# xiyichen/morphablediffusion

Hardware: AMD Instinct MI355X
Metric: multi-view denoising steps/sec (N=16 views, 256x256, CFG 2.0, DDIM-50 step) (higher is better)
Workload: dtype f16; 1 GPU; synthetic sample (FaceScape-FLAME-sized mesh, 5023 vertices before voxel de-duplication): N=16 target views, 256x256 (latent 32x32), perspective cameras, full-width UNet (916.9M params, random init), CFG 2.0, one denoise_apply per step; views_per_gpu=16, batch_view_num=16, parallelism=single GPU

## Files before the change

include/mvd.h:

```cpp
#ifndef MVD_H
#define MVD_H
#include <stddef.h>
#include <stdint.h>

#ifdef __cplusplus
extern "C" {
#endif

typedef struct mvd_ctx mvd_ctx;

typedef struct {
  int image_size;
  int in_channels;
  int out_channels;
  int model_channels;
  int num_res_blocks;
  int channel_mult[4];
  int num_heads;
  int context_dim;
  int volume_dims[4];
  int attention_levels;
} mvd_unet_config;

typedef struct {
// ... 132 lines not shown
int mvd_denoise_views_ms(mvd_ctx* ctx, int B, const int* slots, const float* x_noisy, const float* x_input, const float* clip,
                         const int64_t* timesteps, const float* t_embed, const float* v_embed, const int32_t* view_idx, int TN,
                         float cfg_scale, const float* noise, float s1m, float sqrt_at, float c_x, float c_d, float c_c, float c_n,
                         float* x0_hist, int first, float* eps_out, float* x_next, void* stream);

int mvd_op_cfg_ms(const float* eps_c, const float* eps_u, float scale, const float* x, const float* noise, float s1m, float sqrt_at,
                  float c_x, float c_d, float c_c, float c_n, float* x0_hist, int first, float* eps_out, float* x_next, size_t n,
                  void* stream);
int mvd_op_adamw_ex(float* p, const float* g, float* m, float* v, float* e, size_t n, float lr, float beta1, float beta2, float eps,
                    float wd, int step, float inv_scale, float max_grad_norm, float ema_decay, float* norm_out, void* stream);
int mvd_op_conv(mvd_ctx* ctx, const float* x_nchw, int B, int Cin, int H, int W, const float* w, const float* bias,
                int Cout, int ksize, int stride, int upsample, const float* resid_nchw, float* out_nchw, int force_splitk,
                void* stream);
int mvd_op_linear(mvd_ctx* ctx, const float* a, int M, int K, const float* w, const float* bias, int N, int geglu,
                  const float* resid, int a_half, int force_splitk, float* out, void* stream);
int mvd_op_group_norm(mvd_ctx* ctx, const float* x_nchw, int B, int C, int HW, int groups, const float* gamma,
                      const float* beta, float eps, int act, float* out_nchw, void* stream);
int mvd_op_layer_norm(mvd_ctx* ctx, const float* x, int rows, int C, const float* gamma, const float* beta, float* out,
                      void* stream);
int mvd_op_attention(mvd_ctx* ctx, const float* q, const float* k, const float* v, int B, int T, int heads, int d,
                     float* out, void* stream);
int mvd_op_depth_attn(mvd_ctx* ctx, const float* qk, const float* context, const float* fill_row, int n_cond, int HW, int D, int Cc,
                      int heads, int ldx, int split, int nfill, int check_only, float* out, float* hi_out, void* stream);
int mvd_op_conv3d(mvd_ctx* ctx, const float* x_ncdhw, int B, int Cin, int D, int H, int W, const float* w,
                  const float* bias, int Cout, int stride, int transposed, const float* resid, float* out, void* stream);
int mvd_op_attention_bwd(mvd_ctx* ctx, const float* q, const float* k, const float* v, const float* d_out, int B, int T, int heads,
                         int d, float* dq, float* dk, float* dv, void* stream);
int mvd_op_group_norm_bwd(mvd_ctx* ctx, const float* x, const float* dy, int B, int rows, int C, int groups, const float* gamma,
                          const float* beta, float eps, int act, float* dx, float* dgamma, float* dbeta, void* stream);
int mvd_op_layer_norm_bwd(mvd_ctx* ctx, const float* x, const float* dy, int rows, int C, const float* gamma, float* dx,
                          float* dgamma, float* dbeta, void* stream);
int mvd_op_conv_bwd(mvd_ctx* ctx, int kind, int ksize, int B, int Cin, int H, int W, int Cout, const float* x, int x_f16,
                    const float* w, const float* dy, int xp, int accum, int need_din, int poison, float* dx, float* dw, float* db,
                    void* stream);
int mvd_op_linear_bwd(mvd_ctx* ctx, int B, int rows, int K, int N, const float* x, int x_f16, const float* w, const float* bias,
                      const float* dy, int geglu, int dx_f16, int staged, int xp, int accum, int poison, float* dx, float* dw,
                      float* db, void* stream);
int mvd_op_conv3d_bwd(mvd_ctx* ctx, int kind, int B, int Cin, int D, int H, int W, int Cout, const float* x, int x_f16,
                      const float* w, const float* dy, int accum, int poison, float* dx, float* dw, float* db, void* stream);
int mvd_op_tgemm(mvd_ctx* ctx, int M, int N, int K, const float* a, int a_f16, int a_trans, long lda, const float* b, int b_f16,
                 int b_trans, long ldb, float* out, int ldc, int accum, int xp, int poison, void* stream);
int mvd_op_st_tail(mvd_ctx* ctx, int C, int rows, int T, const float* ao, const float* xin, const float* rowbias,
                   const float* w_ao, const float* b_ao, const float* ln_g, const float* ln_b, const float* w1, const float* b1,
                   const float* w2, const float* b2, const float* w_po, const float* b_po, const float* resid, float* out,
                   int flags, int iters, float* ms_out, void* stream);
int mvd_op_st_head(mvd_ctx* ctx, int rows, int xp, const float* n0, const float* w_pi, const float* b_pi, const float* ln_g,
// ... 17 lines not shown
```

morphablediffusion_amd/csrc/c_api.hip:

```cpp
#include <array>
#include <dlfcn.h>
#include <stdlib.h>
#include <string.h>

#include <algorithm>
#include <string>
#include <utility>
#include <vector>

#include "engine.h"
#include "rowchain.h"

static thread_local std::string g_err;
int mvd_fail(const char* msg) {
  g_err = msg ? msg : "unknown error";
  return -1;
}
const char* mvd_error_text() { return g_err.c_str(); }

namespace {

__global__ void split_rows_to_f32_kernel(const half_t* in, int rows, int C, float* out) {
  for (size_t i = (size_t)blockIdx.x * blockDim.x + threadIdx.x; i < (size_t)rows * C; i += (size_t)gridDim.x * blockDim.x) {
    const size_t r = i / C, c = i % C;
// ... 1312 lines not shown
  split = split ? 1 : 0;
  const int W4 = 4 * Cc, wz = split ? 3 : 1;
  const size_t npix = (size_t)n_cond * HW, rows = npix + nfill, crows = npix * D;
  half_t* cn = ws_alloc<half_t>(c, crows * ldx + 8);
  half_t* z = ws_alloc<half_t>(c, (rows + 1) * W4 * wz);
  half_t* fr = ws_alloc<half_t>(c, (size_t)W4 * 3);
  WS_CHECK(cn && z && fr);
  HIP_CHECK_RET(hipMemsetAsync(cn, 0xFF, (crows * ldx + 8) * sizeof(half_t), s));
  HIP_CHECK_RET(hipMemsetAsync(z, 0xFF, (rows + 1) * W4 * wz * sizeof(half_t), s));
  if (crows) hipLaunchKernelGGL(rows_f32_to_f16_ld_kernel, dim3(nblk(crows * Cc)), dim3(256), 0, s, context, crows, Cc, cn, ldx);
  if (nfill > 0) {
    if (split) RET_IF(launch_rows_f32_to_f16_split(fill_row, W4, 1, W4, fr, s));
    else RET_IF(launch_f32_to_f16(fill_row, fr, W4, s));
  }
  RET_IF(launch_depth_attn(qk, cn, z, n_cond, HW, D, Cc, heads, s, split, nfill, nfill > 0 ? fr : nullptr, ldx));
  const size_t n = (rows + 1) * W4;
  if (split) {
    hipLaunchKernelGGL(split_rows_to_f32_kernel, dim3(nblk(n)), dim3(256), 0, s, z, (int)(rows + 1), W4, out);
    if (hi_out) hipLaunchKernelGGL(rows_f16_ld_to_f32_kernel, dim3(nblk(n)), dim3(256), 0, s, z, rows + 1, W4, 3 * W4, hi_out);
  } else {
    hipLaunchKernelGGL(f16_to_f32_kernel, dim3(nblk(n)), dim3(256), 0, s, z, out, n);
  }
  HIP_CHECK_RET(hipGetLastError());
  return 0;
}

int mvd_op_attention_bwd(mvd_ctx* c, const float* q, const float* k, const float* v, const float* d_out, int B, int T, int heads, int d,
                         float* dq, float* dk, float* dv, void* stream) {
  if (c && hipSetDevice(c->device) != hipSuccess) return mvd_fail("hipSetDevice failed");
  if (!c) return mvd_fail("null context");
  hipStream_t s = S(stream);
  WsScope ws_scope(c);
  const int C = heads * d, rows = B * T;
  half_t* qkv = ws_alloc<half_t>(c, (size_t)rows * 3 * C);
  half_t* o = ws_alloc<half_t>(c, (size_t)rows * C);
  half_t* do16 = ws_alloc<half_t>(c, (size_t)rows * C);
  half_t* dqkv = ws_alloc<half_t>(c, (size_t)rows * 3 * C);
  float* lse = ws_alloc<float>(c, (size_t)B * heads * T);
  float* delta = ws_alloc<float>(c, (size_t)B * heads * T);
  float* tmp = ws_alloc<float>(c, (size_t)rows * 3 * C);
  WS_CHECK(qkv && o && do16 && dqkv && lse && delta && tmp);
  hipLaunchKernelGGL(pack_qkv_rows_kernel, dim3(nblk((size_t)rows * C)), dim3(256), 0, s, q, k, v, rows, C, qkv);
  RET_IF(launch_attention(qkv, 3 * C, qkv + 2 * C, 3 * C, o, C, B, T, heads, d, s));
  RET_IF(bwd_cast_rows(d_out, C, rows, C, C, do16, s));
  RET_IF(bwd_attention(qkv, 3 * C, o, do16, C, dqkv, 3 * C, lse, delta, B, T, heads, d, s));
  hipLaunchKernelGGL(f16_to_f32_kernel, dim3(nblk((size_t)rows * 3 * C)), dim3(256), 0, s, dqkv, tmp, (size_t)rows * 3 * C);
// ... 375 lines not shown
```

morphablediffusion_amd/csrc/common.h:

```cpp
#pragma once
#include <hip/hip_runtime.h>
#include <hip/hip_fp16.h>
#include <stdint.h>

#include "env.h"

#ifdef MVD_BF16
typedef __bf16 half_t;
#define MVD_MFMA_32x32x16 __builtin_amdgcn_mfma_f32_32x32x16_bf16
#define MVD_MFMA_16x16x32 __builtin_amdgcn_mfma_f32_16x16x32_bf16
#define MVD_DTYPE_NAME "bf16"
#else
typedef _Float16 half_t;
#define MVD_MFMA_32x32x16 __builtin_amdgcn_mfma_f32_32x32x16_f16
#define MVD_MFMA_16x16x32 __builtin_amdgcn_mfma_f32_16x16x32_f16
#define MVD_DTYPE_NAME "f16"
#endif
typedef half_t h8 __attribute__((ext_vector_type(8)));
typedef half_t h4 __attribute__((ext_vector_type(4)));
typedef half_t h2 __attribute__((ext_vector_type(2)));
typedef float f32x16 __attribute__((ext_vector_type(16)));
typedef float f32x4 __attribute__((ext_vector_type(4)));

#define MVD_MAX_TAPS 27
// ... 116 lines not shown
int launch_gn_group(const float* x, int ld, int B, int rows, int C, int G, const float* preadd, int pld, const float* gamma,
                    const float* beta, float eps, int act, half_t* out, int ldo, hipStream_t s, int split = 0,
                    int nslab = 1, size_t slab_stride = 0, const float* bias2 = nullptr, const float* resid = nullptr, int ldr = 0,
                    float* mat = nullptr, int ldm = 0);
int launch_layernorm(const float* x, int rows, int C, const float* gamma, const float* beta, float eps,
                     half_t* out, hipStream_t s, half_t* raw = nullptr, int ld_raw = 0);
bool layernorm_slabs_takes(int C);
int launch_layernorm_slabs(const float* slabs, int nslab, size_t slab_stride, int rows, int C, const float* bias, const float* rowbias,
                           int rb_ld, int T, const float* resid, int ldr, float* mat, const float* gamma, const float* beta, float eps,
                           half_t* out, hipStream_t s, half_t* raw = nullptr, int ld_raw = 0);
int launch_layernorm_f32(const float* x, long ldx, int rows, int C, const float* gamma, const float* beta, float eps,
                         float* out, hipStream_t s);
int launch_attention(const half_t* qk, int ldqk, const half_t* v, int ldv, half_t* out, int ldo, int B, int T, int heads,
                     int d, hipStream_t s, int Tstride = 0);
int launch_clip_patches(const float* img, int B, int H, int W, int S, int P, int Kp, half_t* out, hipStream_t s);
int launch_clip_tokens(const float* pe, const float* cls, const float* pos, int B, int T, int Tp, int C, float* x,
                       hipStream_t s);
int launch_scale_copy(const float* src, size_t n, float k, float* dst, hipStream_t s);
int launch_softmax_rows(const float* s, long rows, int cols, half_t* p, hipStream_t st);
int launch_softmax_rows_f32(const float* s, long rows, int cols, float* p, hipStream_t st);
int launch_depth_attn(const float* qk, const half_t* ctxn, half_t* z, int n_cond, int HW, int D, int Cc, int heads,
                      hipStream_t s, int split = 0, int nfill = 0, const half_t* fill_row = nullptr, int ldx = 0);
int depth_attn_check(int D, int Cc, int heads, int ldx, int nfill);
int launch_small_linear(const float* a, int lda, int rows, int K, const half_t* w, const float* bias, int N,
                        int act_in, float* out, int ldo, int accumulate, hipStream_t s);
int launch_timestep_embedding(const int64_t* t, int B, int dim, float* out, hipStream_t s);
int launch_nchw_to_nhwc(const float* in, int B, int C, int HW, float* out, int ldo, int cpad, hipStream_t s);
int launch_nhwc_to_nchw(const float* in, int ld, int B, int C, int HW, float* out, hipStream_t s);
int launch_pack_weight(const float* src, int N, int Cin, int taps, int transposed, int geglu, half_t* dst,
                       hipStream_t s, int cin_src = -1, int xp = 0);
int launch_rows_f32_to_f16_split(const float* in, int lda, long rows, int C, half_t* out, hipStream_t s);
int launch_permute_geglu_bias(const float* src, int N, float* dst, hipStream_t s);
int launch_f32_to_f16(const float* in, half_t* out, size_t n, hipStream_t s);
int launch_rows_f32_to_f16(const float* in, int lda, long rows, int C, half_t* out, hipStream_t s);
int launch_pack_upconv_weight(const float* src, int N, int Cin, half_t* dst, hipStream_t s);
int launch_fill_rows_f16(half_t* out, int ld, int rows, const half_t* vec, int n, hipStream_t s);
int launch_fold_qk(const float* wq, const float* wk, int heads, int hd, int Cc, int I, float scale, half_t* out,
                   hipStream_t s, float* out32 = nullptr);
int launch_fold_ov(const float* wo, const float* wv, int heads, int hd, int Cc, int I, half_t* out, hipStream_t s,
                   float* out32 = nullptr);
int launch_fold_mm(const float* a, int lda, const float* b, int ldb, int M, int N, int K, half_t* out16, int ldc, float* out32,
                   hipStream_t s);
int launch_relu_beta_tile(const float* beta, int Cc, int heads, half_t* out, hipStream_t s, int split = 0);
int launch_cfg_ddim(const float* eps_c, const float* eps_u, float scale, const float* x, const float* noise,
                    float sqrt_one_minus_at, float sqrt_at, float sqrt_aprev, float dir_coef, float sigma,
                    float* eps_out, float* x_prev, size_t n, hipStream_t s);
// ... 127 lines not shown
```

morphablediffusion_amd/csrc/engine_unet.hip:

```cpp
#include <string.h>

#include <algorithm>

#include "engine.h"

namespace {

void igemm_init(IGemm& g) {
  memset(&g, 0, sizeof(g));
  g.alpha = 1.0f;
  g.sz = g.sy = g.sx = 1;
  g.out_linear = 1;
  g.Z = g.Y = g.X = g.B = 1;
  g.IZ = g.IY = g.IX = 1;
  g.PZ = g.PY = g.PX = 1;
  for (int i = 0; i < MVD_MAX_TAPS; ++i) g.tap[i] = igemm_tap(0, 0, 0, i);
}

void igemm_fill(IGemm& g, const GemmArgs& ga) {
  g.a = ga.a;
  g.a_f32 = ga.a_f32;
  g.lda = ga.lda;
  g.Cin = ga.w->Cin;
  g.cin_alg = ga.w->xp ? ga.w->cin_l : ga.w->Cin;
// ... 752 lines not shown
  half_t* z = ws_alloc<half_t>(c, (size_t)rows * 4 * Cc * wz);
  float* o = ws_alloc<float>(c, (size_t)rows * I);
  float* o2 = ws_alloc<float>(c, (size_t)rows * I);
  WS_CHECK(p && pn && z && o && o2);
  const size_t slab_elems = (size_t)rows * I;
  auto offer_slabs = [&](GemmArgs& ga, int* sk, int ldo) {
    *sk = 1;
    if (!mvd_env().cond_defer || f.train || !gn_group_eligible(I, HW, I, 8, 0, ldo)) return;
    const size_t nsl = rows > 8192 ? 4 : 16;
    ga.slabs = ws_alloc<float>(c, nsl * slab_elems);
    ga.slabs_cap = ga.slabs ? nsl * slab_elems : 0;
    ga.sk_used = sk;
  };
  GemmArgs g;
  int skd = 1;
  g.a = in.p; g.a_f32 = 1; g.lda = in.ld; g.w = &d.proj_in; g.out = p; g.ldc = I;
  offer_slabs(g, &skd, xq ? 3 * I : I);
  RET_IF(run_linear(c, g, Bx, rows, f.s));
  if (skd > 1)
    RET_IF(run_group_norm(c, g.slabs, I, Bx, HW, d.gn_in, 8, 1e-5f, ACT_SILU, nullptr, pn, xq ? 3 * I : I, f.s, 0, xq, skd, slab_elems,
                          d.proj_in.bias));
  else
    RET_IF(run_group_norm(c, p, I, Bx, HW, d.gn_in, 8, 1e-5f, ACT_SILU, nullptr, pn, xq ? 3 * I : I, f.s, 0, xq));
  if (f.n_ctx > 0) {
    float* qk = ws_alloc<float>(c, (size_t)crow * 4 * Cc);
    half_t* cn = cond_idx >= 0 && f.cn_pre[cond_idx] ? nullptr : ws_alloc<half_t>(c, (size_t)crow * D * Cc);
    WS_CHECK(qk && (cn || (cond_idx >= 0 && f.cn_pre[cond_idx])));
    g = GemmArgs();
    g.a = pn; g.lda = xq ? 3 * I : I; g.w = &d.wqk; g.out = qk; g.ldc = 4 * Cc; g.use_bias = false;
    RET_IF(run_linear(c, g, f.n_ctx, crow, f.s));
    const half_t* cnp = cond_idx >= 0 ? f.cn_pre[cond_idx] : nullptr;
    if (cnp) {
      HIP_CHECK_RET(hipStreamWaitEvent(f.s, c->ev_cond[cond_idx], 0));
      cn = const_cast<half_t*>(cnp);
    } else if (ctx_fold_ok(f, d, HW, D, level)) {
      if (f.ctx_side) HIP_CHECK_RET(hipStreamWaitEvent(f.s, c->ev_ctx, 0));
      RET_IF(ctx_fold(f, d, HW, D, level, cn, f.s));
    } else {
      if (f.ctx_side) HIP_CHECK_RET(hipStreamWaitEvent(f.s, c->ev_ctx, 0));
      float* pc = ws_alloc<float>(c, (size_t)crow * D * Cc);
      WS_CHECK(pc);
      g = GemmArgs();
      g.a = f.src[level].p; g.a_f32 = f.src[level].f32; g.lda = Cc; g.w = &d.proj_ctx; g.out = pc; g.ldc = Cc; g.use_bias = false;
      RET_IF(run_linear(c, g, f.n_ctx, crow * D, f.s));
      RET_IF(run_group_norm(c, pc, Cc, f.n_ctx, D * HW, d.gn_ctx, 8, 1e-5f, ACT_RELU, nullptr, cn, Cc, f.s));
    }
    {
      ProbeScope ps(c, f.s, "depth_attn_kernel", 4.0 * crow * (double)D * 4 * Cc,
                    (double)crow * D * Cc * 2.0 + (double)crow * 4 * Cc * 6.0);
      RET_IF(launch_depth_attn(qk, cn, z, f.n_ctx, HW, D, Cc, 4, f.s, xo, rows - crow, d.relu_beta, cnp ? f.cn_ld[cond_idx] : Cc));
    }
  } else if (Bx > f.n_ctx) {
    RET_IF(launch_fill_rows_f16(z + (size_t)crow * 4 * Cc * wz, 4 * Cc * wz, rows - crow, d.relu_beta, 4 * Cc * wz, f.s));
  }
  g = GemmArgs();
  g.a = z; g.lda = 4 * Cc * wz; g.w = &d.wov; g.out = o; g.ldc = I; g.use_bias = false;
  offer_slabs(g, &skd, x1 ? 3 * I : I);
  RET_IF(run_linear(c, g, Bx, rows, f.s));
  if (skd > 1)
    RET_IF(run_group_norm(c, g.slabs, I, Bx, HW, d.gn_o1, 8, 1e-5f, ACT_RELU, nullptr, pn, x1 ? 3 * I : I, f.s, 0, x1, skd, slab_elems));
  else
    RET_IF(run_group_norm(c, o, I, Bx, HW, d.gn_o1, 8, 1e-5f, ACT_RELU, nullptr, pn, x1 ? 3 * I : I, f.s, 0, x1));
  g = GemmArgs();
  g.a = pn; g.lda = x1 ? 3 * I : I; g.w = &d.conv1; g.out = o2; g.ldc = I; g.use_bias = false;
  offer_slabs(g, &skd, x2 ? 3 * I : I);
  RET_IF(run_conv2d(c, g, Bx, H, W, 1, 0, f.s));
  if (skd > 1)
    RET_IF(run_group_norm(c, g.slabs, I, Bx, HW, d.gn_o2, 8, 1e-5f, ACT_RELU, nullptr, pn, x2 ? 3 * I : I, f.s, 0, x2, skd, slab_elems));
  else
    RET_IF(run_group_norm(c, o2, I, Bx, HW, d.gn_o2, 8, 1e-5f, ACT_RELU, nullptr, pn, x2 ? 3 * I : I, f.s, 0, x2));
  g = GemmArgs();
  g.a = pn; g.lda = x2 ? 3 * I : I; g.w = &d.conv2; g.out = out.p; g.ldc = out.ld; g.use_bias = false; g.resid = in.p; g.ldr = in.ld;
  RET_IF(run_conv2d(c, g, Bx, H, W, 1, 0, f.s));
  if (use_const) {
    ProbeScope ps(c, f.s, "cond_const_add", 0.0, (double)n_free * HW * d.dim * 8.0);
    RET_IF(launch_add_image_rows(in.p + (size_t)crow * in.ld, in.ld, c->cond_const[cond_idx].k, d.dim, n_free, HW,
                                 out.p + (size_t)crow * out.ld, out.ld, f.s));
  }
  return 0;
}

// ... 532 lines not shown
```

morphablediffusion_amd/csrc/env.h:

```cpp
#pragma once

#define MVD_ENV_TABLE(PROCESS, ENGINE, CALL, PROCESS_CALL) \
   \
  ENGINE(off, halo, "MVD_NO_HALO", true, "3x3 convs on the gather kernel instead of the LDS-halo / conv3x kernels") \
  PROCESS_CALL(off, conv3x, "MVD_NO_CONV3X", true, "no conv3x fragment streams: 3x3 ResBlock convs on the LDS-halo kernel") \
  PROCESS(off, up_conv3x, "MVD_NO_UP_CONV3X", true, "the 4x4 -> 8x8 upsample conv as the 9-tap GEMM on the fp32 source, not upsample + conv3x") \
  PROCESS(off, gemm_dma, "MVD_NO_GEMM_DMA", true, "GEMMs / 1x1 convs on the older register-staged igemm kernel, not the LDS-DMA kernel") \
  PROCESS(num, dense_min_m, "MVD_DENSE_MIN_M", 64, "fewest rows routed to the LDS-DMA kernel (2 views per rank: 7.08 ms at 512, 6.97 ms at 64)") \
  PROCESS(off, plain, "MVD_NO_PLAIN", true, "general row mapping for plain GEMMs instead of the PLAIN instantiations") \
  PROCESS(on, old_plan, "MVD_OLD_PLAN", false, "k-step cost model (gemm_dma_plan) instead of gemm_dma_plan_us for plain GEMMs") \
  PROCESS(on, igemm_f32_bn128, "MVD_IGEMM_F32_BN128", false, "fp32 sources on 128-column tiles where 160 is picked (32768 x 960 x 320: 48 vs 37 us)") \
  PROCESS(on, bm128, "MVD_BM128", false, "offer the planner the four-wave 128-row tiles: measured, lost (profiles/r06_b_bm_sweep.txt)") \
  PROCESS(on, bm128_off, "MVD_NO_BM128", false, "overrides MVD_BM128: the 128-row tiles stay off") \
  PROCESS(num, dense_bn, "MVD_DENSE_BN", 0, "sweep (tools/gemm_plan_sweep.py): column-tile width of the dense launches, 0 = planner's") \
  PROCESS(num, dense_sk, "MVD_DENSE_SK", 0, "sweep: split-K of the dense launches, 0 = planner's") \
  PROCESS(num, dense_bm, "MVD_DENSE_BM", 0, "sweep: 128 = four-wave row tiles with MVD_DENSE_BN, else 256") \
  PROCESS(num, halo_bn, "MVD_HALO_BN", 0, "sweep (tools/conv_bench3.py): column width of the LDS-halo kernel, 0 = planner's") \
  PROCESS(num, halo_sk, "MVD_HALO_SK", 0, "sweep: split over 64-channel chunks of the LDS-halo kernel, 0 = planner's") \
  PROCESS(off, parity_batch, "MVD_NO_PARITY_BATCH", true, "one launch per output-parity class of the transposed / upsample convs, not one for all") \
  PROCESS(num, par_walk_min, "MVD_PAR_WALK_MIN", 0, "tiles from which a workgroup walks the parity classes, 0 = never (profiles/r06_y_ab_pwalk.txt: nothing)") \
  PROCESS(off, xcd_cols, "MVD_NO_XCD_COLS", true, "row-tile-major XCD walk always, never the column-major one (common.h: xcd_prefers_cols)") \
  PROCESS(off, attn_xcd, "MVD_ATTN_NO_XCD", true, "attention with the pre-remap workgroup order") \
   \
  PROCESS(num, defer_max, "MVD_DEFER_MAX", 16, "largest split a consumer takes as slabs (4 = the round-3 limit)") \
  PROCESS(off, defer_reduce, "MVD_NO_DEFER_REDUCE", true, "ResBlock conv1 with its own reduce pass; also turns off ln_defer and cond_defer") \
  PROCESS(off, cond_defer, "MVD_NO_COND_DEFER", true, "the DepthTransformer's GEMMs in front of a GroupNorm with their reduce passes") \
  PROCESS(on, ln_defer, "MVD_LN_DEFER", false, "LayerNorm sums the split-K slabs of proj_in / to_out (profiles/r06_g_ab_ln_defer.txt: no time gained)") \
  PROCESS(off, carry, "MVD_NO_CARRY", true, "a block's last GEMM reduces its own slabs instead of leaving them to the next block's GroupNorm") \
   \
  PROCESS(on, gn_two_pass, "MVD_GN_TWO_PASS", false, "two-pass GroupNorm everywhere; also turns off defer_reduce, cond_defer and out_conv_f32") \
  PROCESS(on, skip_side, "MVD_SKIP_SIDE", false, "the ResBlock's 1x1 skip conv on a helper stream (profiles/r06_z_ab_skip_side.txt: nothing)") \
  PROCESS(off, rowchain, "MVD_NO_ROWCHAIN", true, "the transformer block behind the attention as layered GEMMs, not the row-chain kernel") \
  PROCESS(num, rowchain_min_rows, "MVD_ROWCHAIN_MIN_ROWS", 16384, "fewest rows that take the row-chain kernel") \
  PROCESS(off, rowhead, "MVD_NO_ROWHEAD", true, "proj_in, LayerNorm1 and q | k | v as separate launches, not the row-head kernel") \
  PROCESS(off, xp_fuse, "MVD_NO_XP_FUSE", true, "extended-precision proj_in / proj_out as separate GEMMs beside the row kernels") \
  PROCESS(off, ffp, "MVD_NO_FFP", true, "FF2 and proj_out as two GEMMs, not one over [gg | t2]") \
  PROCESS(on, ln_scalar, "MVD_LN_SCALAR", false, "element-per-thread LayerNorm (also keeps FF2 and proj_out apart)") \
  PROCESS(off, ctx_fold, "MVD_NO_CTX_FOLD", true, "GroupNorm(proj_context(volume)) materialised, not folded into two GEMM passes") \
  PROCESS(off, ctx_group, "MVD_NO_CTX_GROUP", true, "context fold block by block, not once per level") \
  PROCESS(off, cond_const, "MVD_NO_COND_CONST", true, "DepthTransformer over all samples, context-free ones included (profiles/r06_i_ab_cond_const.txt)") \
  PROCESS(off, conv_in_f32, "MVD_NO_CONV_IN_F32", true, "the input conv on the MFMA forms, not in exact fp32 on the vector ALU") \
  PROCESS(off, out_conv_f32, "MVD_NO_OUT_CONV_F32", true, "the output head on the MFMA forms, not GroupNorm + conv in exact fp32") \
  PROCESS(off, side_stream, "MVD_NO_SIDE_STREAM", true, "context volumes and folds on the caller's stream") \
  PROCESS(off, side_emb, "MVD_NO_SIDE_EMB", true, "the timestep-embedding GEMMs on the caller's stream") \
  PROCESS(on, one_way_fork, "MVD_ONE_WAY_FORK", false, "side-stream fork without the acknowledgement: the round-1 race on demand (DESIGN.md section 4, tools/det_fork.sh)") \
   \
  PROCESS(off, fused_enc, "MVD_NO_FUSED_ENC", true, "the 2-D target encoder layer by layer, not as one launch") \
  CALL(one, bn_loop, "MVD_BN_LOOP", false, "the looped BatchNorm + ReLU kernel; tests/test_gpu_train.py flips it for its bit-identity check") \
  CALL(one, sparse_valu, "MVD_SPARSE_VALU", false, "read when sparse-conv weights are built: one-site-per-workgroup kernels and the scatter-form data gradient") \
  CALL(num, xp, "MVD_XP", precision_level, "overrides the engine's extended-precision level when the policy is applied") \
  PROCESS(on, stage_scalar, "MVD_STAGE_SCALAR", false, "element-per-thread staging kernels of the backward pass (profiles/r04_m_*)") \
  PROCESS(on, gn_bwd_one_block, "MVD_GN_BWD_ONE_BLOCK", false, "mvd_op_group_norm_bwd: one workgroup per (sample, group), not the slabbed form") \
  PROCESS(one, repack_one_stream, "MVD_REPACK_STREAMS", false, "=1: the training re-pack on one stream, not four") \
   \
  PROCESS(on, plan_debug, "MVD_PLAN_DEBUG", false, "print every dense plan as a [plan] line") \
  PROCESS(on, layer_timing, "MVD_LAYER_TIMING", false, "per-GEMM event time (tools/layer_step.py); synchronises every launch") \
  PROCESS(on, debug_sum, "MVD_DEBUG_SUM", false, "bit checksums of the step's buffers: which differ between repeats?") \
  PROCESS(on, mesh_timing, "MVD_MESH_TIMING", false, "host phases of set_mesh / set_samples") \
  PROCESS(on, cond_bwd_timing, "MVD_COND_BWD_TIMING", false, "host-side enqueue time of each conditioner-backward phase")

#include <stdlib.h>

// ... 45 lines not shown
```

morphablediffusion_amd/engine.py:

```python
import collections
import ctypes as C
import os
from typing import Dict, Optional

import torch

from . import lib as L
from .spec import UNetConfig, VolumeConfig


def _stream():
    return torch.cuda.current_stream().cuda_stream


def _f32(t, device):
    return t.detach().to(device=device, dtype=torch.float32).contiguous()


IncompatibleKeys = collections.namedtuple("IncompatibleKeys", ["missing_keys", "unexpected_keys"])
MAX_SAMPLE_SLOTS = 64


def _level_dims(d, s):
    out = []
# ... 745 lines not shown
                                          _stream()))
        return out

    def op_depth_attn(self, qk, ctx, fill_row=None, nfill=0, split=False, ldx=0, heads=4, return_hi=False):
        dev = self.device
        qk, ctx = _f32(qk, dev), _f32(ctx, dev)
        n_cond, D, HW, Cc = ctx.shape
        fr = None if fill_row is None else _f32(fill_row, dev)
        err = self.op_depth_attn_check(D, Cc, heads=heads, ldx=ldx, nfill=nfill)
        if err is not None:
            raise L.MvdError(err)
        if qk.numel() != n_cond * HW * 4 * Cc or (nfill > 0 and (fr is None or fr.numel() != 4 * Cc)):
            raise ValueError("op_depth_attn: qk / fill_row do not match the context's shape")
        out = torch.empty(n_cond * HW + nfill + 1, 4 * Cc, device=dev, dtype=torch.float32)
        hi = torch.empty_like(out) if split and return_hi else None
        L.check(self.lib.mvd_op_depth_attn(self._ctx, L.ptr(qk), L.ptr(ctx), L.ptr(fr), n_cond, HW, D, Cc, heads, ldx, bool(split),
                                           nfill, 0, L.ptr(out), L.ptr(hi), _stream()))
        return (out, hi) if return_hi else out

    def op_depth_attn_check(self, D, Cc, heads=4, ldx=0, nfill=0):
        rc = self.lib.mvd_op_depth_attn(self._ctx, None, None, None, 0, 1, D, Cc, heads, ldx, 0, nfill, 1, None, None, _stream())
        return None if rc == 0 else self.lib.mvd_last_error().decode()

    def op_attention_bwd(self, q, k, v, d_out, heads):
        dev = self.device
        q, k, v, d_out = _f32(q, dev), _f32(k, dev), _f32(v, dev), _f32(d_out, dev)
        B, T, Cc = q.shape
        dq, dk, dv = torch.empty_like(q), torch.empty_like(q), torch.empty_like(q)
        L.check(self.lib.mvd_op_attention_bwd(self._ctx, L.ptr(q), L.ptr(k), L.ptr(v), L.ptr(d_out), B, T, heads, Cc // heads,
                                              L.ptr(dq), L.ptr(dk), L.ptr(dv), _stream()))
        return dq, dk, dv

    def op_group_norm_bwd(self, x, dy, groups, gamma, beta, eps, act=0):
        dev = self.device
        x, dy, g, b = _f32(x, dev), _f32(dy, dev), _f32(gamma, dev), _f32(beta, dev)
        B, rows, Cc = x.shape
        dx, dg, db = torch.empty_like(x), torch.empty_like(g), torch.empty_like(g)
        L.check(self.lib.mvd_op_group_norm_bwd(self._ctx, L.ptr(x), L.ptr(dy), B, rows, Cc, groups, L.ptr(g), L.ptr(b), eps,
                                               act, L.ptr(dx), L.ptr(dg), L.ptr(db), _stream()))
        return dx, dg, db

    def op_layer_norm_bwd(self, x, dy, gamma):
        dev = self.device
        x, dy, g = _f32(x, dev), _f32(dy, dev), _f32(gamma, dev)
        dx, dg, db = torch.empty_like(x), torch.empty_like(g), torch.empty_like(g)
        L.check(self.lib.mvd_op_layer_norm_bwd(self._ctx, L.ptr(x), L.ptr(dy), x.shape[0], x.shape[1], L.ptr(g), L.ptr(dx), L.ptr(dg),
# ... 136 lines not shown
```

Before: 78.50 steps/s.

## Fuse DepthTransformer wqk GEMM, depth attention and wov GEMM into one kernel

Adds a depth_core kernel that, per tile of pixels, computes the wqk projection with MFMA into LDS, runs the softmax attention over depth samples of the context volume, and applies the wov projection, all in one launch. It runs by default in inference when the context rows and shapes fit (Cc 64/128, D within one LDS pass). This removes the fp32 qk and f16 z intermediates in global memory and two extra launches. In exchange the slab split-k path for the wov GEMM is skipped, weights are re-read per block, and LDS use limits occupancy. Also adds a C and Python op with a built-in timing loop for testing.

```diff
diff --git a/include/mvd.h b/include/mvd.h
--- a/include/mvd.h
+++ b/include/mvd.h
@@ -178,6 +178,9 @@
                      float* out, void* stream);
 int mvd_op_depth_attn(mvd_ctx* ctx, const float* qk, const float* context, const float* fill_row, int n_cond, int HW, int D, int Cc,
                       int heads, int ldx, int split, int nfill, int check_only, float* out, float* hi_out, void* stream);
+int mvd_op_depth_core(mvd_ctx* ctx, const float* pn, const float* wqk, const float* wov, const float* context, int n_cond, int HW,
+                      int D, int Cc, int I, int ldx, int xq, int xo, int layered, int check_only, int iters, float* ms_out,
+                      float* out, void* stream);
 int mvd_op_conv3d(mvd_ctx* ctx, const float* x_ncdhw, int B, int Cin, int D, int H, int W, const float* w,
                   const float* bias, int Cout, int stride, int transposed, const float* resid, float* out, void* stream);
 int mvd_op_attention_bwd(mvd_ctx* ctx, const float* q, const float* k, const float* v, const float* d_out, int B, int T, int heads,
diff --git a/morphablediffusion_amd/csrc/c_api.hip b/morphablediffusion_amd/csrc/c_api.hip
--- a/morphablediffusion_amd/csrc/c_api.hip
+++ b/morphablediffusion_amd/csrc/c_api.hip
@@ -1358,6 +1358,67 @@
     hipLaunchKernelGGL(f16_to_f32_kernel, dim3(nblk(n)), dim3(256), 0, s, z, out, n);
   }
   HIP_CHECK_RET(hipGetLastError());
+  return 0;
+}
+
+int mvd_op_depth_core(mvd_ctx* c, const float* pn, const float* wqk, const float* wov, const float* context, int n_cond, int HW, int D,
+                      int Cc, int I, int ldx, int xq, int xo, int layered, int check_only, int iters, float* ms_out, float* out,
+                      void* stream) {
+  if (c && hipSetDevice(c->device) != hipSuccess) return mvd_fail("hipSetDevice failed");
+  if (!c) return mvd_fail("null context");
+  if (depth_core_check(D, Cc, I, xq, xo, ldx)) return -1;
+  if (check_only) return 0;
+  if (n_cond <= 0 || HW <= 0 || !pn || !wqk || !wov || !context || !out || (iters > 0 && !ms_out)) return mvd_fail("op_depth_core: bad argument");
+  hipStream_t s = S(stream);
+  WsScope ws_scope(c);
+  if (ldx == 0) ldx = Cc;
+  xq = xq ? 1 : 0;
+  xo = xo ? 1 : 0;
+  const int W4 = 4 * Cc, Kq = xq ? 3 * I : I, Kz = xo ? 3 * W4 : W4;
+  const size_t npix = (size_t)n_cond * HW, crows = npix * D;
+  half_t* cn = ws_alloc<half_t>(c, crows * ldx + 8);
+  half_t* p16 = ws_alloc<half_t>(c, npix * Kq);
+  half_t* wq16 = ws_alloc<half_t>(c, (size_t)W4 * Kq);
+  half_t* wo16 = ws_alloc<half_t>(c, (size_t)I * Kz);
+  float* qk = layered ? ws_alloc<float>(c, npix * W4) : nullptr;
+  half_t* z = layered ? ws_alloc<half_t>(c, npix * Kz) : nullptr;
+  WS_CHECK(cn && p16 && wq16 && wo16 && (!layered || (qk && z)));
+  HIP_CHECK_RET(hipMemsetAsync(cn, 0xFF, (crows * ldx + 8) * sizeof(half_t), s));
+  HIP_CHECK_RET(hipMemsetAsync(out, 0xFF, (npix + 1) * I * sizeof(float), s));
+  hipLaunchKernelGGL(rows_f32_to_f16_ld_kernel, dim3(nblk(crows * Cc)), dim3(256), 0, s, context, crows, Cc, cn, ldx);
+  HIP_CHECK_RET(hipGetLastError());
+  if (xq) RET_IF(launch_rows_f32_to_f16_split(pn, I, (long)npix, I, p16, s));
+  else RET_IF(launch_f32_to_f16(pn, p16, npix * I, s));
+  RET_IF(launch_pack_weight(wqk, W4, Kq, 1, 0, 0, wq16, s, I, xq));
+  RET_IF(launch_pack_weight(wov, I, Kz, 1, 0, 0, wo16, s, W4, xo));
+  ConvW cq, co;
+  cq.w = wq16; cq.N = W4; cq.Cin = Kq; cq.xp = xq; cq.cin_l = I;
+  co.w = wo16; co.N = I; co.Cin = Kz; co.xp = xo; co.cin_l = W4;
+  auto run = [&]() -> int {
+    if (!layered) return launch_depth_core(p16, Kq, wq16, wo16, cn, ldx, out, n_cond, HW, D, Cc, I, xq, xo, s);
+    GemmArgs g;
+    g.a = p16; g.lda = Kq; g.w = &cq; g.out = qk; g.ldc = W4; g.use_bias = false;
+    RET_IF(run_linear(c, g, n_cond, (int)npix, s));
+    RET_IF(launch_depth_attn(qk, cn, z, n_cond, HW, D, Cc, 4, s, xo, 0, nullptr, ldx));
+    g = GemmArgs();
+    g.a = z; g.lda = Kz; g.w = &co; g.out = out; g.ldc = I; g.use_bias = false;
+    return run_linear(c, g, n_cond, (int)npix, s);
+  };
+  RET_IF(run());
+  if (iters > 0) {
+    hipEvent_t e0, e1;
+    HIP_CHECK_RET(hipEventCreate(&e0));
+    HIP_CHECK_RET(hipEventCreate(&e1));
+    HIP_CHECK_RET(hipEventRecord(e0, s));
+    for (int i = 0; i < iters; ++i) RET_IF(run());
+    HIP_CHECK_RET(hipEventRecord(e1, s));
+    HIP_CHECK_RET(hipEventSynchronize(e1));
+    float ms = 0.f;
+    HIP_CHECK_RET(hipEventElapsedTime(&ms, e0, e1));
+    hipEventDestroy(e0);
+    hipEventDestroy(e1);
+    *ms_out = ms / (float)iters;
+  }
   return 0;
 }
 
diff --git a/morphablediffusion_amd/csrc/common.h b/morphablediffusion_amd/csrc/common.h
--- a/morphablediffusion_amd/csrc/common.h
+++ b/morphablediffusion_amd/csrc/common.h
@@ -162,6 +162,11 @@
 int launch_depth_attn(const float* qk, const half_t* ctxn, half_t* z, int n_cond, int HW, int D, int Cc, int heads,
                       hipStream_t s, int split = 0, int nfill = 0, const half_t* fill_row = nullptr, int ldx = 0);
 int depth_attn_check(int D, int Cc, int heads, int ldx, int nfill);
+int launch_depth_core(const half_t* pn, int lda, const half_t* wqk, const half_t* wov, const half_t* ctxn, int ldx, float* o,
+                      int n_cond, int HW, int D, int Cc, int I, int xq, int xo, hipStream_t s);
+const char* depth_core_refusal(int D, int Cc, int I, int xq, int xo, int ldx);
+bool depth_core_one_pass(int D, int Cc);
+int depth_core_check(int D, int Cc, int I, int xq, int xo, int ldx);
 int launch_small_linear(const float* a, int lda, int rows, int K, const half_t* w, const float* bias, int N,
                         int act_in, float* out, int ldo, int accumulate, hipStream_t s);
 int launch_timestep_embedding(const int64_t* t, int B, int dim, float* out, hipStream_t s);
diff --git a/morphablediffusion_amd/csrc/engine_unet.hip b/morphablediffusion_amd/csrc/engine_unet.hip
--- a/morphablediffusion_amd/csrc/engine_unet.hip
+++ b/morphablediffusion_amd/csrc/engine_unet.hip
@@ -798,14 +798,20 @@
                           d.proj_in.bias));
   else
     RET_IF(run_group_norm(c, p, I, Bx, HW, d.gn_in, 8, 1e-5f, ACT_SILU, nullptr, pn, xq ? 3 * I : I, f.s, 0, xq));
+  const half_t* cnp = f.n_ctx > 0 && cond_idx >= 0 ? f.cn_pre[cond_idx] : nullptr;
+  const int cn_ld = cnp ? f.cn_ld[cond_idx] : Cc;
+  const bool core = mvd_env().depth_core && !f.train && !c->train_mode && f.n_ctx > 0 && rows == crow &&
+                    crow >= mvd_env().depth_core_min_rows && !(Cc > 64 && (xq || xo)) && depth_core_one_pass(D, Cc) &&
+                    !depth_core_refusal(D, Cc, I, xq, xo, cn_ld);
   if (f.n_ctx > 0) {
-    float* qk = ws_alloc<float>(c, (size_t)crow * 4 * Cc);
-    half_t* cn = cond_idx >= 0 && f.cn_pre[cond_idx] ? nullptr : ws_alloc<half_t>(c, (size_t)crow * D * Cc);
-    WS_CHECK(qk && (cn || (cond_idx >= 0 && f.cn_pre[cond_idx])));
-    g = GemmArgs();
-    g.a = pn; g.lda = xq ? 3 * I : I; g.w = &d.wqk; g.out = qk; g.ldc = 4 * Cc; g.use_bias = false;
-    RET_IF(run_linear(c, g, f.n_ctx, crow, f.s));
-    const half_t* cnp = cond_idx >= 0 ? f.cn_pre[cond_idx] : nullptr;
+    float* qk = core ? nullptr : ws_alloc<float>(c, (size_t)crow * 4 * Cc);
+    half_t* cn = cnp ? nullptr : ws_alloc<half_t>(c, (size_t)crow * D * Cc);
+    WS_CHECK((qk || core) && (cn || cnp));
+    if (!core) {
+      g = GemmArgs();
+      g.a = pn; g.lda = xq ? 3 * I : I; g.w = &d.wqk; g.out = qk; g.ldc = 4 * Cc; g.use_bias = false;
+      RET_IF(run_linear(c, g, f.n_ctx, crow, f.s));
+    }
     if (cnp) {
       HIP_CHECK_RET(hipStreamWaitEvent(f.s, c->ev_cond[cond_idx], 0));
       cn = const_cast<half_t*>(cnp);
@@ -821,18 +827,25 @@
       RET_IF(run_linear(c, g, f.n_ctx, crow * D, f.s));
       RET_IF(run_group_norm(c, pc, Cc, f.n_ctx, D * HW, d.gn_ctx, 8, 1e-5f, ACT_RELU, nullptr, cn, Cc, f.s));
     }
-    {
+    if (core) {
+      ProbeScope ps(c, f.s, "depth_core_kernel", 4.0 * crow * (double)D * 4 * Cc + 2.0 * 2.0 * crow * (double)I * 4 * Cc,
+                    (double)crow * D * Cc * 2.0 + (double)crow * I * 6.0 + 2.0 * 2.0 * I * 4 * Cc);
+      RET_IF(launch_depth_core(pn, xq ? 3 * I : I, d.wqk.w, d.wov.w, cn, cn_ld, o, f.n_ctx, HW, D, Cc, I, xq, xo, f.s));
+    } else {
       ProbeScope ps(c, f.s, "depth_attn_kernel", 4.0 * crow * (double)D * 4 * Cc,
                     (double)crow * D * Cc * 2.0 + (double)crow * 4 * Cc * 6.0);
-      RET_IF(launch_depth_attn(qk, cn, z, f.n_ctx, HW, D, Cc, 4, f.s, xo, rows - crow, d.relu_beta, cnp ? f.cn_ld[cond_idx] : Cc));
+      RET_IF(launch_depth_attn(qk, cn, z, f.n_ctx, HW, D, Cc, 4, f.s, xo, rows - crow, d.relu_beta, cn_ld));
     }
   } else if (Bx > f.n_ctx) {
     RET_IF(launch_fill_rows_f16(z + (size_t)crow * 4 * Cc * wz, 4 * Cc * wz, rows - crow, d.relu_beta, 4 * Cc * wz, f.s));
   }
   g = GemmArgs();
-  g.a = z; g.lda = 4 * Cc * wz; g.w = &d.wov; g.out = o; g.ldc = I; g.use_bias = false;
-  offer_slabs(g, &skd, x1 ? 3 * I : I);
-  RET_IF(run_linear(c, g, Bx, rows, f.s));
+  skd = 1;
+  if (!core) {
+    g.a = z; g.lda = 4 * Cc * wz; g.w = &d.wov; g.out = o; g.ldc = I; g.use_bias = false;
+    offer_slabs(g, &skd, x1 ? 3 * I : I);
+    RET_IF(run_linear(c, g, Bx, rows, f.s));
+  }
   if (skd > 1)
     RET_IF(run_group_norm(c, g.slabs, I, Bx, HW, d.gn_o1, 8, 1e-5f, ACT_RELU, nullptr, pn, x1 ? 3 * I : I, f.s, 0, x1, skd, slab_elems));
   else
diff --git a/morphablediffusion_amd/csrc/env.h b/morphablediffusion_amd/csrc/env.h
--- a/morphablediffusion_amd/csrc/env.h
+++ b/morphablediffusion_amd/csrc/env.h
@@ -38,6 +38,8 @@
   PROCESS(on, ln_scalar, "MVD_LN_SCALAR", false, "element-per-thread LayerNorm (also keeps FF2 and proj_out apart)") \
   PROCESS(off, ctx_fold, "MVD_NO_CTX_FOLD", true, "GroupNorm(proj_context(volume)) materialised, not folded into two GEMM passes") \
   PROCESS(off, ctx_group, "MVD_NO_CTX_GROUP", true, "context fold block by block, not once per level") \
+  PROCESS(off, depth_core, "MVD_NO_DEPTH_CORE", true, "the DepthTransformer core as wqk GEMM, depth attention and wov GEMM, not the one-launch depth_core kernel") \
+  PROCESS(num, depth_core_min_rows, "MVD_DEPTH_CORE_MIN_ROWS", 512, "fewest context rows (n_ctx * H * W) that take the depth_core kernel") \
   PROCESS(off, cond_const, "MVD_NO_COND_CONST", true, "DepthTransformer over all samples, context-free ones included (profiles/r06_i_ab_cond_const.txt)") \
   PROCESS(off, conv_in_f32, "MVD_NO_CONV_IN_F32", true, "the input conv on the MFMA forms, not in exact fp32 on the vector ALU") \
   PROCESS(off, out_conv_f32, "MVD_NO_OUT_CONV_F32", true, "the output head on the MFMA forms, not GroupNorm + conv in exact fp32") \
diff --git a/morphablediffusion_amd/csrc/k_depthcore.hip b/morphablediffusion_amd/csrc/k_depthcore.hip
--- /dev/null
+++ b/morphablediffusion_amd/csrc/k_depthcore.hip
@@ -0,0 +1,318 @@
+#include "common.h"
+
+namespace {
+
+constexpr int DCORE_CTX_BYTES = 40 * 1024;
+
+template <int CC, int TP>
+struct DCore {
+  static constexpr int W4 = 4 * CC, I = 2 * CC, MR = TP / 16, XLD = CC + 8;
+  static constexpr int QLD = W4 + 4;
+  static constexpr int R1 = TP * QLD * 4;
+  static constexpr int DCMAX = DCORE_CTX_BYTES / (TP * XLD * 2);
+  static int dc(int D) { return D < DCMAX ? D : DCMAX; }
+  static int lds(int D, int xq) {
+    const int kq = xq ? 3 * I : I, r3a = TP * (kq + 8) * 2, r3b = TP * dc(D) * XLD * 2;
+    return R1 + TP * D * 16 + (r3a > r3b ? r3a : r3b);
+  }
+};
+
+template <int MR, int NT, int U, class KA, class KW>
+__device__ __forceinline__ void dcore_gemm(f32x4 (&acc)[MR][NT], const half_t* arow, int ald, const half_t* wrow, long wld, int S, KA ka,
+                                           KW kw) {
+  h8 b[U][NT][2];
+#pragma unroll
+  for (int u = 0; u < U; ++u)
+#pragma unroll
+    for (int n = 0; n < NT; ++n) {
+      const half_t* w = wrow + n * 16 * wld + kw(u);
+      b[u][n][0] = *(const h8*)w;
+      b[u][n][1] = *(const h8*)(w + 8);
+    }
+  for (int s0 = 0; s0 < S; s0 += U) {
+#pragma unroll
+    for (int u = 0; u < U; ++u) {
+      const int s = s0 + u;
+      h8 a[MR][2];
+#pragma unroll
+      for (int m = 0; m < MR; ++m) {
+        const half_t* ap = arow + m * 16 * ald + ka(s);
+        a[m][0] = *(const h8*)ap;
+        a[m][1] = *(const h8*)(ap + 8);
+      }
+#pragma unroll
+      for (int m = 0; m < MR; ++m)
+#pragma unroll
+        for (int n = 0; n < NT; ++n) {
+          acc[m][n] = MVD_MFMA_16x16x32(a[m][0], b[u][n][0], acc[m][n], 0, 0, 0);
+          acc[m][n] = MVD_MFMA_16x16x32(a[m][1], b[u][n][1], acc[m][n], 0, 0, 0);
+        }
+      if (s + U < S) {
+#pragma unroll
+        for (int n = 0; n < NT; ++n) {
+          const half_t* w = wrow + n * 16 * wld + kw(s + U);
+          b[u][n][0] = *(const h8*)w;
+          b[u][n][1] = *(const h8*)(w + 8);
+        }
+      }
+    }
+  }
+}
+
+template <int CC, int TP>
+__global__ __launch_bounds__(256) void depth_core_kernel(const half_t* __restrict__ pn, int lda, const half_t* __restrict__ wqk,
+                                                         const half_t* __restrict__ wov, const half_t* __restrict__ ctxn, int ldx,
+                                                         float* __restrict__ o, int npix, int HW, int D, int xq, int xo) {
+#if defined(__HIP_DEVICE_COMPILE__)
+  using K = DCore<CC, TP>;
+  constexpr int W4 = K::W4, I = K::I, MR = K::MR, XLD = K::XLD, QLD = K::QLD;
+  extern __shared__ __attribute__((aligned(16))) char smem[];
+  const int tid = threadIdx.x, lane = tid & 63, wave = tid >> 6;
+  const int fr = lane & 15, fq = lane >> 4;
+  const int p0 = blockIdx.x * TP;
+  const int Kq = xq ? 3 * I : I, Kz = xo ? 3 * W4 : W4;
+  const int DC = D < K::DCMAX ? D : K::DCMAX;
+  float* sQK = (float*)smem;
+  half_t* sZ = (half_t*)smem;
+  float* sA = (float*)(smem + K::R1);
+  half_t* sPN = (half_t*)(smem + K::R1 + TP * D * 16);
+  half_t* sX = sPN;
+  const int pld = Kq + 8, zld = (xo ? 2 : 1) * W4 + 8;
+
+  constexpr int SB = 3;
+  {
+    const int cpr = Kq >> 3, total = TP * cpr;
+    for (int base = tid; base < total; base += SB * 256) {
+      h8 v[SB];
+#pragma unroll
+      for (int u = 0; u < SB; ++u) {
+        const int idx = base + u * 256 < total ? base + u * 256 : total - 1;
+        const int j = idx / cpr, ch = idx - j * cpr, pix = p0 + j < npix ? p0 + j : npix - 1;
+        v[u] = *(const h8*)(pn + (long)pix * lda + ch * 8);
+      }
+#pragma unroll
+      for (int u = 0; u < SB; ++u) {
+        const int idx = base + u * 256, j = idx / cpr, ch = idx - j * cpr;
+        if (idx < total) *(h8*)(sPN + j * pld + ch * 8) = p0 + j < npix ? v[u] : (h8)(half_t)0;
+      }
+    }
+  }
+  __syncthreads();
+
+  {
+    constexpr int NT = CC / 16;
+    f32x4 acc[MR][NT];
+#pragma unroll
+    for (int m = 0; m < MR; ++m)
+#pragma unroll
+      for (int n = 0; n < NT; ++n) acc[m][n] = (f32x4){0.f, 0.f, 0.f, 0.f};
+    const half_t* wrow = wqk + (long)(wave * CC + fr) * Kq + fq * 16;
+    const half_t* arow = sPN + fr * pld + fq * 16;
+    auto kk = [&](int st) { const int k = st * 64 + I; return k < Kq ? k : k - Kq; };
+    dcore_gemm<MR, NT, 2>(acc, arow, pld, wrow, (long)Kq, Kq / 64, kk, kk);
+#pragma unroll
+    for (int m = 0; m < MR; ++m)
+#pragma unroll
+      for (int n = 0; n < NT; ++n)
+#pragma unroll
+        for (int r = 0; r < 4; ++r) sQK[(m * 16 + fq * 4 + r) * QLD + wave * CC + n * 16 + fr] = acc[m][n][r];
+  }
+  __syncthreads();
+
+  constexpr int cprx = CC / 8, NB = (K::DCMAX * TP * cprx + 255) / 256;
+  h8 cv[NB];
+  auto ctx_load = [&](int d0, int nd) {
+    const int total = nd * TP * cprx;
+#pragma unroll
+    for (int u = 0; u < NB; ++u) {
+      const int idx = tid + u * 256 < total ? tid + u * 256 : total - 1;
+      const int ch = idx % cprx, rest = idx / cprx, j = rest % TP, dl = rest / TP;
+      const int pix = p0 + j < npix ? p0 + j : npix - 1, b = pix / HW, p = pix - b * HW;
+      cv[u] = *(const h8*)(ctxn + (((long)b * D + d0 + dl) * HW + p) * ldx + ch * 8);
+    }
+  };
+  auto ctx_store = [&](int nd) {
+    const int total = nd * TP * cprx;
+#pragma unroll
+    for (int u = 0; u < NB; ++u) {
+      const int idx = tid + u * 256, ch = idx % cprx, rest = idx / cprx, j = rest % TP, dl = rest / TP;
+      if (idx < total) *(h8*)(sX + (j * DC + dl) * XLD + ch * 8) = p0 + j < npix ? cv[u] : (h8)(half_t)0;
+    }
+  };
+  auto pass_nd = [&](int d0) { return D - d0 < DC ? D - d0 : DC; };
+
+  ctx_load(0, pass_nd(0));
+  for (int d0 = 0; d0 < D; d0 += DC) {
+    const int nd = pass_nd(d0);
+    if (d0) __syncthreads();
+    ctx_store(nd);
+    __syncthreads();
+    const int dn = d0 + DC < D ? d0 + DC : (D > DC ? 0 : d0);
+    ctx_load(dn, pass_nd(dn));
+    for (int e = tid; e < TP * 4 * nd; e += 256) {
+      const int dl = e % nd, jh = e / nd, h = jh & 3, j = jh >> 2;
+      const half_t* xr = sX + (j * DC + dl) * XLD;
+      const float* qr = sQK + j * QLD + h * CC;
+      float acc = 0.f;
+#pragma unroll 4
+      for (int c = 0; c < CC; c += 8) {
+        const h8 xv = *(const h8*)(xr + c);
+        const float4 qa = *(const float4*)(qr + c), qb = *(const float4*)(qr + c + 4);
+        acc += (float)xv[0] * qa.x + (float)xv[1] * qa.y + (float)xv[2] * qa.z + (float)xv[3] * qa.w +
+               (float)xv[4] * qb.x + (float)xv[5] * qb.y + (float)xv[6] * qb.z + (float)xv[7] * qb.w;
+      }
+      sA[(j * D + d0 + dl) * 4 + h] = acc;
+    }
+  }
+  __syncthreads();
+
+  {
+    constexpr int PP = 256 / (4 * TP);
+    const int part = tid % PP, jh = tid / PP, h = jh & 3, j = jh >> 2;
+    float* ar = sA + j * D * 4 + h;
+    float mx = -INFINITY;
+    for (int d = part; d < D; d += PP) mx = fmaxf(mx, ar[d * 4]);
+#pragma unroll
+    for (int s = 1; s < PP; s <<= 1) mx = fmaxf(mx, __shfl_xor(mx, s));
+    float sum = 0.f;
+    for (int d = part; d < D; d += PP) {
+      const float e = __expf(ar[d * 4] - mx);
+      ar[d * 4] = e;
+      sum += e;
+    }
+#pragma unroll
+    for (int s = 1; s < PP; s <<= 1) sum += __shfl_xor(sum, s);
+    const float inv = 1.0f / sum;
+    for (int d = part; d < D; d += PP) ar[d * 4] *= inv;
+  }
+  __syncthreads();
+
+  {
+    constexpr int cpr = CC / 8, NI = TP * 4 * cpr / 256;
+    float acc[NI][8];
+#pragma unroll
+    for (int i = 0; i < NI; ++i)
+#pragma unroll
+      for (int k = 0; k < 8; ++k) acc[i][k] = 0.f;
+    for (int d0 = 0; d0 < D; d0 += DC) {
+      const int nd = D - d0 < DC ? D - d0 : DC;
+      if (D > DC) {
+        __syncthreads();
+        ctx_store(nd);
+        __syncthreads();
+        const int dn = d0 + DC < D ? d0 + DC : d0;
+        ctx_load(dn, pass_nd(dn));
+      }
+#pragma unroll
+      for (int i = 0; i < NI; ++i) {
+        const int it = tid + i * 256, oct = it % cpr, jh = it / cpr, h = jh & 3, j = jh >> 2;
+        const half_t* xr = sX + j * DC * XLD + oct * 8;
+        const float* ar = sA + (j * D + d0) * 4 + h;
+        for (int dl = 0; dl < nd; ++dl) {
+          const h8 xv = *(const h8*)(xr + dl * XLD);
+          const float a = ar[dl * 4];
+#pragma unroll
+          for (int k = 0; k < 8; ++k) acc[i][k] += a * (float)xv[k];
+        }
+      }
+    }
+#pragma unroll
+    for (int i = 0; i < NI; ++i) {
+      const int it = tid + i * 256, oct = it % cpr, jh = it / cpr, h = jh & 3, j = jh >> 2;
+      h8 hi;
+#pragma unroll
+      for (int k = 0; k < 8; ++k) hi[k] = (half_t)acc[i][k];
+      half_t* zr = sZ + j * zld + h * CC + oct * 8;
+      *(h8*)zr = hi;
+      if (xo) {
+        h8 lo;
+#pragma unroll
+        for (int k = 0; k < 8; ++k) lo[k] = (half_t)(acc[i][k] - (float)hi[k]);
+        *(h8*)(zr + W4) = lo;
+      }
+    }
+  }
+  __syncthreads();
+
+  {
+    constexpr int NT = I / 64;
+    f32x4 acc[MR][NT];
+#pragma unroll
+    for (int m = 0; m < MR; ++m)
+#pragma unroll
+      for (int n = 0; n < NT; ++n) acc[m][n] = (f32x4){0.f, 0.f, 0.f, 0.f};
+    const int c0 = wave * (I / 4);
+    const half_t* wrow = wov + (long)(c0 + fr) * Kz + fq * 16;
+    const half_t* arow = sZ + fr * zld + fq * 16;
+    constexpr int SPS = W4 / 64;
+    auto seg = [&](int st) { return xo ? (st / SPS + 1) % 3 : 0; };
+    auto ka = [&](int st) { return (seg(st) == 1 ? W4 : 0) + (st % SPS) * 64; };
+    auto kw = [&](int st) { return seg(st) * W4 + (st % SPS) * 64; };
+    dcore_gemm<MR, NT, 4>(acc, arow, zld, wrow, (long)Kz, Kz / 64, ka, kw);
+#pragma unroll
+    for (int m = 0; m < MR; ++m)
+#pragma unroll
+      for (int r = 0; r < 4; ++r) {
+        const int pix = p0 + m * 16 + fq * 4 + r;
+        if (pix < npix) {
+#pragma unroll
+          for (int n = 0; n < NT; ++n) o[(long)pix * I + c0 + n * 16 + fr] = acc[m][n][r];
+        }
+      }
+  }
+#endif
+}
+
+template <int CC, int TP>
+int depth_core_go(const half_t* pn, int lda, const half_t* wqk, const half_t* wov, const half_t* ctxn, int ldx, float* o, int npix,
+                  int HW, int D, int xq, int xo, hipStream_t s) {
+  using K = DCore<CC, TP>;
+  const int lds = K::lds(D, xq);
+  static bool attr_done[MVD_MAX_DEVICES] = {false};
+  bool& attr_set = attr_done[mvd_current_device()];
+  if (!attr_set) {
+    HIP_CHECK_RET(hipFuncSetAttribute((const void*)depth_core_kernel<CC, TP>, hipFuncAttributeMaxDynamicSharedMemorySize, 160 * 1024));
+    attr_set = true;
+  }
+  hipLaunchKernelGGL((depth_core_kernel<CC, TP>), dim3(cdiv(npix, TP)), dim3(256), lds, s, pn, lda, wqk, wov, ctxn, ldx, o, npix, HW,
+                     D, xq, xo);
+  HIP_CHECK_RET(hipGetLastError());
+  return 0;
+}
+
+}
+
+const char* depth_core_refusal(int D, int Cc, int I, int xq, int xo, int ldx) {
+  if (Cc != 64 && Cc != 128) return "depth_core: context widths 64 and 128 only (others take the layered path)";
+  if (I != 2 * Cc) return "depth_core: the inner width must be 2 * Cc";
+  if (D < 1 || D > 64) return "depth_core: 1 <= D <= 64";
+  if (ldx == 0) ldx = Cc;
+  if (ldx < Cc || (ldx & 7)) return "depth_core: context rows must be 16-byte aligned and at least Cc wide";
+  const int lds = Cc == 64 ? DCore<64, 32>::lds(D, xq) : DCore<128, 16>::lds(D, xq);
+  if (lds > 160 * 1024) return "depth_core: LDS budget exceeded";
+  (void)xo;
+  return nullptr;
+}
+
+bool depth_core_one_pass(int D, int Cc) { return D <= (Cc == 64 ? DCore<64, 32>::DCMAX : DCore<128, 16>::DCMAX); }
+
+int depth_core_check(int D, int Cc, int I, int xq, int xo, int ldx) {
+  const char* why = depth_core_refusal(D, Cc, I, xq, xo, ldx);
+  return why ? mvd_fail(why) : 0;
+}
+
+int launch_depth_core(const half_t* pn, int lda, const half_t* wqk, const half_t* wov, const half_t* ctxn, int ldx, float* o,
+                      int n_cond, int HW, int D, int Cc, int I, int xq, int xo, hipStream_t s) {
+  if (depth_core_check(D, Cc, I, xq, xo, ldx)) return -1;
+  if (ldx == 0) ldx = Cc;
+  xq = xq ? 1 : 0;
+  xo = xo ? 1 : 0;
+  if (lda < (xq ? 3 : 1) * I || (lda & 7)) return mvd_fail("depth_core: pn rows must be 16-byte aligned and hold the whole operand");
+  if (((uintptr_t)pn | (uintptr_t)wqk | (uintptr_t)wov | (uintptr_t)ctxn | (uintptr_t)o) & 15)
+    return mvd_fail("depth_core: operands must be 16-byte aligned");
+  if (n_cond < 0 || HW <= 0 || (long)n_cond * HW > 0x7fffffffL - 64) return mvd_fail("depth_core: bad row count");
+  const int npix = n_cond * HW;
+  if (npix == 0) return 0;
+  if (Cc == 64) return depth_core_go<64, 32>(pn, lda, wqk, wov, ctxn, ldx, o, npix, HW, D, xq, xo, s);
+  return depth_core_go<128, 16>(pn, lda, wqk, wov, ctxn, ldx, o, npix, HW, D, xq, xo, s);
+}
diff --git a/morphablediffusion_amd/engine.py b/morphablediffusion_amd/engine.py
--- a/morphablediffusion_amd/engine.py
+++ b/morphablediffusion_amd/engine.py
@@ -791,6 +791,27 @@
         rc = self.lib.mvd_op_depth_attn(self._ctx, None, None, None, 0, 1, D, Cc, heads, ldx, 0, nfill, 1, None, None, _stream())
         return None if rc == 0 else self.lib.mvd_last_error().decode()
 
+    def op_depth_core(self, pn, wqk, wov, ctx, xq=False, xo=False, ldx=0, layered=False, iters=0):
+        dev = self.device
+        pn, wqk, wov, ctx = _f32(pn, dev), _f32(wqk, dev), _f32(wov, dev), _f32(ctx, dev)
+        n_cond, D, HW, Cc = ctx.shape
+        I = pn.shape[-1]
+        err = self.op_depth_core_check(D, Cc, I, xq=xq, xo=xo, ldx=ldx)
+        if err is not None:
+            raise L.MvdError(err)
+        if pn.numel() != n_cond * HW * I or wqk.numel() != 4 * Cc * I or wov.numel() != 4 * Cc * I:
+            raise ValueError("op_depth_core: pn / wqk / wov do not match the context's shape")
+        out = torch.empty(n_cond * HW + 1, I, device=dev, dtype=torch.float32)
+        ms = C.c_float(0)
+        L.check(self.lib.mvd_op_depth_core(self._ctx, L.ptr(pn), L.ptr(wqk), L.ptr(wov), L.ptr(ctx), n_cond, HW, D, Cc, I, ldx, bool(xq),
+                                           bool(xo), bool(layered), 0, iters, C.byref(ms), L.ptr(out), _stream()))
+        return (out, ms.value) if iters > 0 else out
+
+    def op_depth_core_check(self, D, Cc, I, xq=False, xo=False, ldx=0):
+        rc = self.lib.mvd_op_depth_core(self._ctx, None, None, None, None, 0, 1, D, Cc, I, ldx, bool(xq), bool(xo), 0, 1, 0, None, None,
+                                        _stream())
+        return None if rc == 0 else self.lib.mvd_last_error().decode()
+
     def op_attention_bwd(self, q, k, v, d_out, heads):
         dev = self.device
         q, k, v, d_out = _f32(q, dev), _f32(k, dev), _f32(v, dev), _f32(d_out, dev)
```

After: 78.18 steps/s. No clear change (-0.4%).
